# leoelm/Bayesian_inference_for_NN

Hardware: NVIDIA B200
Metric: posterior_grad_evals_per_s (higher is better)
Workload: dtype f32 (tensor-core products on two int8 fixed-point slices per operand, kind::i8, exact int32 accumulate; f32 everywhere else)

## Files before the change

### bayesian_inference_for_nn_b200/csrc/tc_fused.cuh

```cuda
#pragma once
#include "tc_layer2.cuh"

namespace pyb {

constexpr int TF_THREADS = 384;
template <int CP> struct TfCfg {
  static constexpr int STAGES = 5;
  static constexpr int W2_BYTES = 2 * 256 * CP * 4;
  static constexpr int ZX_BYTES = 2 * CP * 128 * 4;
  static constexpr int SMEM = STAGES * TP_STAGE_BYTES + 1024  + 1024  + 2048  +
                              128  + W2_BYTES + ZX_BYTES;
  static constexpr int SMEM_I8 = SMEM + 4096;
};
__device__ __forceinline__ void tc_ld_16x256b_x4_raw(uint32_t taddr, uint32_t* r) {
  asm volatile(
      "tcgen05.ld.sync.aligned.16x256b.x4.b32 "
      "{%0, %1, %2, %3, %4, %5, %6, %7, %8, %9, %10, %11, %12, %13, %14, %15}, [%16];"
      : "=r"(r[0]), "=r"(r[1]), "=r"(r[2]), "=r"(r[3]), "=r"(r[4]), "=r"(r[5]), "=r"(r[6]), "=r"(r[7]), "=r"(r[8]),
        "=r"(r[9]), "=r"(r[10]), "=r"(r[11]), "=r"(r[12]), "=r"(r[13]), "=r"(r[14]), "=r"(r[15])
      : "r"(taddr)
      : "memory");
}
__device__ __forceinline__ void tc_mma_i8_pair(uint32_t tmem_d, uint64_t adesc, uint64_t bdesc, uint32_t idesc,
                                               uint32_t accumulate) {
  asm volatile(
      "{\n"
      ".reg .pred p;\n"
      "setp.ne.b32 p, %4, 0;\n"
      "tcgen05.mma.cta_group::2.kind::i8 [%0], %1, %2, %3, p;\n"
      "}\n" ::"r"(tmem_d),
      "l"(adesc), "l"(bdesc), "r"(idesc), "r"(accumulate)
      : "memory");
}
__device__ __forceinline__ void slice4_i8(const float* d, float zq, uint32_t& hw, uint32_t& lw) {
  constexpr float M = 12582912.0f;
  uint32_t hb[4], lb[4];
#pragma unroll
  for (int r = 0; r < 4; ++r) {
    const float t = fmaf(d[r], zq, M);
    const float h = t - M;
    const float e = fmaf(d[r], zq, -h);
    const float u = fmaf(e, 254.0f, M);
    hb[r] = __float_as_uint(t);
    lb[r] = __float_as_uint(u);
  }
  hw = __byte_perm(__byte_perm(hb[0], hb[1], 0x0040), __byte_perm(hb[2], hb[3], 0x0040), 0x5410);
  lw = __byte_perm(__byte_perm(lb[0], lb[1], 0x0040), __byte_perm(lb[2], lb[3], 0x0040), 0x5410);
}

__device__ __forceinline__ void tc_ld_16x256b_x4(uint32_t taddr, float* v) {
  uint32_t r[16];
  asm volatile(
      "tcgen05.ld.sync.aligned.16x256b.x4.b32 "
      "{%0, %1, %2, %3, %4, %5, %6, %7, %8, %9, %10, %11, %12, %13, %14, %15}, [%16];"
      : "=r"(r[0]), "=r"(r[1]), "=r"(r[2]), "=r"(r[3]), "=r"(r[4]), "=r"(r[5]), "=r"(r[6]), "=r"(r[7]), "=r"(r[8]),
        "=r"(r[9]), "=r"(r[10]), "=r"(r[11]), "=r"(r[12]), "=r"(r[13]), "=r"(r[14]), "=r"(r[15])
      : "r"(taddr)
      : "memory");
#pragma unroll
  for (int i = 0; i < 16; ++i) v[i] = __uint_as_float(r[i]);
}
template <int CP>
__device__ __forceinline__ int w2_slot(int h, int c) {
  return ((((h >> 3) * 2 + (h & 1)) * (CP / 4) + (c >> 2)) * 4 + ((h >> 1) & 3)) * 4 + (c & 3);
}
__device__ __forceinline__ void split_pair(float x0, float x1, uint32_t& hw, uint32_t& lw) {
  const __nv_bfloat162 hp = __floats2bfloat162_rn(x0, x1);
  hw = *reinterpret_cast<const uint32_t*>(&hp);
  const __nv_bfloat162 lp = __floats2bfloat162_rn(x0 - __uint_as_float(hw << 16), x1 - __uint_as_float(hw & 0xffff0000u));
  lw = *reinterpret_cast<const uint32_t*>(&lp);
}

template <int CP, bool FWD, int I8 = 0>
__global__ void __cluster_dims__(2, 1, 1) __launch_bounds__(TF_THREADS, 1)
tc_g1_layer2_fused(const __grid_constant__ CUtensorMap tmA_hi, const __grid_constant__ CUtensorMap tmA_lo,
                   const __grid_constant__ CUtensorMap tmB_hi, const __grid_constant__ CUtensorMap tmB_lo,
                   const TcGemmParams p, const Layer2Params l2) {
  constexpr int STAGES = TfCfg<CP>::STAGES;
  extern __shared__ uint8_t smem_raw[];
  uint8_t* smem = smem_raw + ((1024u - (smem_u32(smem_raw) & 1023u)) & 1023u);
  uint8_t* stage_base = smem;
  uint64_t* bars = (uint64_t*)(smem + STAGES * TP_STAGE_BYTES);
  uint64_t* full_bar = bars;
  uint64_t* empty_bar = bars + STAGES;
  uint64_t* tmem_full = bars + 2 * STAGES;
  uint64_t* tmem_empty = bars + 2 * STAGES + 2;
  uint32_t* tmem_ptr = (uint32_t*)(bars + 2 * STAGES + 4);
  float* bias_s = (float*)(smem + STAGES * TP_STAGE_BYTES + 1024);
  float* b2_s = bias_s + 512;
  float* W2_s = b2_s + 32;
  float* zx_s = W2_s + 2 * 256 * CP;
  float* cw_s = zx_s + 2 * CP * 128;
  float* zq_s = cw_s + 512;

  const int warp = __shfl_sync(0xffffffffu, (int)(threadIdx.x >> 5), 0), lane = threadIdx.x & 31;
  const uint32_t rank = cluster_ctarank();
  const int cluster_id = blockIdx.x >> 1, n_clusters = gridDim.x >> 1;
  constexpr int KSTAGE = I8 ? 64 : TC_BK;
  const int nk = (p.K + KSTAGE - 1) / KSTAGE;
  const int H = p.H;
  const int half_rows = H >> 1;
  const uint32_t cta_bytes = 2 * TC_A_TILE_BYTES + 2 * (uint32_t)half_rows * TC_BK * 2;

  if (warp == 8 && lane == 0) {
    asm volatile("prefetch.tensormap [%0];" ::"l"(&tmA_hi) : "memory");
    asm volatile("prefetch.tensormap [%0];" ::"l"(&tmA_lo) : "memory");
    asm volatile("prefetch.tensormap [%0];" ::"l"(&tmB_hi) : "memory");
    asm volatile("prefetch.tensormap [%0];" ::"l"(&tmB_lo) : "memory");
  }
  if (warp == 9 && lane == 0) {
    for (int s = 0; s < STAGES; ++s) { mbar_init(&full_bar[s], 1); mbar_init(&empty_bar[s], 1); }
    mbar_init(&tmem_full[0], 1); mbar_init(&tmem_full[1], 1);
    mbar_init(&tmem_empty[0], 16); mbar_init(&tmem_empty[1], 16);
    asm volatile("fence.mbarrier_init.release.cluster;" ::: "memory");
  }
  if (warp == 10) {
    asm volatile("tcgen05.alloc.cta_group::2.sync.aligned.shared::cta.b32 [%0], %1;" ::"r"(smem_u32(tmem_ptr)), "r"(512)
                 : "memory");
    asm volatile("tcgen05.relinquish_alloc_permit.cta_group::2.sync.aligned;" ::: "memory");
  }
  tc_fence_before();
  __syncthreads();
  cluster_sync_all();
  tc_fence_after();
  const uint32_t tmem_base = *tmem_ptr;

  if (warp >= 8) {
   asm volatile("setmaxnreg.dec.sync.aligned.u32 40;");
   if (warp == 8) {
    if (lane == 0) {
      int stage = 0;
      uint32_t phase = 0;
      for (int item = cluster_id; item < p.total_items; item += n_clusters) {
        int b, mp, split;
        tc_decode(p, item, b, mp, split);
        const int arow = p.a_row0 + (mp * 2 + (int)rank) * 128;
        const int brow = b * H + (int)rank * half_rows;
        for (int kc = 0; kc < nk; ++kc) {
          (I8 ? mbar_wait_sleep(&empty_bar[stage], phase ^ 1) : mbar_wait(&empty_bar[stage], phase ^ 1));
          uint8_t* st = stage_base + stage * TP_STAGE_BYTES;
          if (rank == 0) mbar_expect_tx(&full_bar[stage], 2 * cta_bytes);
          const int k0 = kc * KSTAGE;
          tma_load_2d_pair(st, &tmA_hi, &full_bar[stage], k0, arow);
          tma_load_2d_pair(st + TC_A_TILE_BYTES, &tmA_lo, &full_bar[stage], k0, arow);
          tma_load_2d_pair(st + 2 * TC_A_TILE_BYTES, &tmB_hi, &full_bar[stage], k0, brow);
          tma_load_2d_pair(st + 2 * TC_A_TILE_BYTES + 8192, &tmB_lo, &full_bar[stage], k0, brow);
          if (++stage == STAGES) { stage = 0; phase ^= 1; }
        }
      }
    }
  } else if (warp == 9) {
    if (rank == 0 && lane == 0) {
      const uint32_t idesc = (I8 ? (2u << 4) : (1u << 4)) | (1u << 7) | (1u << 10) | ((uint32_t)(H >> 3) << 17) | ((256u >> 4) << 24);
      int stage = 0, it = 0;
      uint32_t phase = 0;
      const int k_tail = p.K - (nk - 1) * KSTAGE;
      for (int item = cluster_id; item < p.total_items; item += n_clusters, ++it) {
        const int acc = I8 ? 0 : (it & 1);
        const uint32_t acc_phase = I8 ? (uint32_t)(it & 1) : (uint32_t)((it >> 1) & 1);
        (I8 ? mbar_wait_sleep(&tmem_empty[acc], acc_phase ^ 1) : mbar_wait(&tmem_empty[acc], acc_phase ^ 1));
        tc_fence_after();
        const uint32_t d = tmem_base + (uint32_t)acc * 256;
        for (int kc = 0; kc < nk; ++kc) {
          (I8 ? mbar_wait_sleep(&full_bar[stage], phase) : mbar_wait(&full_bar[stage], phase));
          tc_fence_after();
          const uint32_t st = smem_u32(stage_base + stage * TP_STAGE_BYTES);
          const int nks = (kc == nk - 1 && k_tail <= KSTAGE / 2) ? 1 : 2;
          for (int ks = 0; ks < nks; ++ks) {
            const uint32_t koff = ks * 32;
            const uint64_t ah = make_smem_desc_sw64(st + koff);
            const uint64_t al = make_smem_desc_sw64(st + TC_A_TILE_BYTES + koff);
            const uint64_t bh = make_smem_desc_sw64(st + 2 * TC_A_TILE_BYTES + koff);
            const uint64_t bl = make_smem_desc_sw64(st + 2 * TC_A_TILE_BYTES + 8192 + koff);
            const uint32_t accum = (kc != 0) || (ks != 0);
            if (I8) {
              tc_mma_i8_pair(d, ah, bh, idesc, accum);
              tc_mma_i8_pair(d + 256, ah, bl, idesc, accum);
              tc_mma_i8_pair(d + 256, al, bh, idesc, 1);
            } else {
              tc_mma_bf16_pair(d, ah, bh, idesc, accum);
              tc_mma_bf16_pair(d, al, bh, idesc, 1);
              tc_mma_bf16_pair(d, ah, bl, idesc, 1);
            }
          }
          tc_commit_pair(&empty_bar[stage]);
          if (++stage == STAGES) { stage = 0; phase ^= 1; }
        }
        tc_commit_pair(&tmem_full[acc]);
      }
    }
   }
  } else {
    asm volatile("setmaxnreg.inc.sync.aligned.u32 232;");
    const int half = warp >> 2;
    const int quad = warp & 3;
    const int g = lane >> 2, t = lane & 3;
    const int eall = threadIdx.x;
    const uint32_t lane_addr = (uint32_t)(quad * 32) << 16;
    const int Hh = H >> 1;
    const int C = l2.C;
    const float invN = l2.scale / (float)l2.N;
    const int r_own = 2 * (t & 1) + (t >> 1);
    const int row_own = quad * 32 + g + 8 * r_own;
    const int pos0 = quad * 32 + 4 * g;
    const int hbase = half * Hh + 2 * t;
    uint16_t* z2_hi = reinterpret_cast<uint16_t*>(l2.z2_hi);
    uint16_t* z2_lo = reinterpret_cast<uint16_t*>(l2.z2_lo);
    for (int i = eall; i < 2 * 256 * CP; i += 256) W2_s[i] = 0.f;
    if (eall < 32) b2_s[eall] = 0.f;
    asm volatile("bar.sync 1, 256;" ::: "memory");
    auto fetch_consts = [&](int item, int buf) {
      int b, mp, split;
      tc_decode(p, item, b, mp, split);
      const float* th = l2.theta + (int64_t)b * l2.P;
      if (eall < H) {
        const int h = eall;
        const float* src = th + l2.w2_off + (int64_t)h * C;
        const uint32_t dst = smem_u32(W2_s + buf * 256 * CP + w2_slot<CP>(h, 0));
#pragma unroll
        for (int c = 0; c < CP; ++c)
          if (c < C)
            asm volatile("cp.async.ca.shared.global [%0], [%1], 4;" ::"r"(dst + (uint32_t)(((c >> 2) * 16 + (c & 3)) * 4)),
                         "l"(src + c) : "memory");
        asm volatile("cp.async.ca.shared.global [%0], [%1], 4;" ::"r"(smem_u32(bias_s + buf * 256 + h)),
                     "l"(p.bias + (int64_t)b * p.bias_stride + h) : "memory");
      }
      if (eall < C)
        asm volatile("cp.async.ca.shared.global [%0], [%1], 4;" ::"r"(smem_u32(b2_s + buf * 16 + eall)),
                     "l"(th + l2.b2_off + eall) : "memory");
      if (I8 && eall < H) {
        asm volatile("cp.async.ca.shared.global [%0], [%1], 4;" ::"r"(smem_u32(cw_s + buf * 256 + eall)),
                     "l"(l2.cw + (int64_t)b * H + eall) : "memory");
        if (I8 == 2 && !FWD)
          asm volatile("cp.async.ca.shared.global [%0], [%1], 4;" ::"r"(smem_u32(zq_s + buf * 256 + eall)),
                       "l"(l2.zq + (int64_t)b * H + eall) : "memory");
      }
    };
    if (cluster_id < p.total_items) fetch_consts(cluster_id, 0);
    int it = 0;
    for (int item = cluster_id; item < p.total_items; item += n_clusters, ++it) {
      int b, mp, split;
      tc_decode(p, item, b, mp, split);
      const int mt = mp * 2 + (int)rank;
      const int cbuf = it & 1;
      const int acc = I8 ? 0 : cbuf;
      const uint32_t acc_phase = I8 ? (uint32_t)(it & 1) : (uint32_t)((it >> 1) & 1);
      float* bs = bias_s + cbuf * 256;
      float* b2b = b2_s + cbuf * 16;
      float* W2b = W2_s + cbuf * 256 * CP;
      float sxr[4] = {0.f, 0.f, 0.f, 0.f};
      if (I8) {
#pragma unroll
        for (int r = 0; r < 4; ++r) {
          const int rg = mt * 128 + quad * 32 + g + 8 * r;
          sxr[r] = rg < p.M_valid ? __ldg(l2.sx + rg) : 0.f;
        }
      }
      asm volatile("cp.async.wait_all;" ::: "memory");
      asm volatile("bar.sync 1, 256;" ::: "memory");
      (I8 ? mbar_wait_sleep(&tmem_full[acc], acc_phase) : mbar_wait(&tmem_full[acc], acc_phase));
      tc_fence_after();
      const int64_t blk_w = (((((int64_t)b * p.out_tiles + mt) * H) + hbase) * 128 + pos0) >> 2;
      uint2* pa_hi = reinterpret_cast<uint2*>(p.out_hi) + blk_w;
      uint2* pa_lo = reinterpret_cast<uint2*>(p.out_lo) + blk_w;
      uint2* pz_hi = reinterpret_cast<uint2*>(l2.zt_hi) + blk_w;
      uint2* pz_lo = reinterpret_cast<uint2*>(l2.zt_lo) + blk_w;
      const float4* w4b = reinterpret_cast<const float4*>(W2b) + (((half * Hh) >> 3) * 2 * (CP / 4)) * 4 + t;
      const float* bsb = bs + hbase;
      const float* cwb = cw_s + cbuf * 256 + hbase;
      const float* zqb = zq_s + cbuf * 256 + hbase;
      uint32_t* pzi_hi = nullptr; uint32_t* pzi_lo = nullptr;
      if (I8 == 2 && !FWD) {
        const int64_t blk_b = ((((int64_t)b * p.out_tiles + mt) * H) + hbase) * 128 + pos0;
        pzi_hi = reinterpret_cast<uint32_t*>(l2.zi_hi + blk_b);
        pzi_lo = reinterpret_cast<uint32_t*>(l2.zi_lo + blk_b);
      }
      float2 z[4][CP / 2];
#pragma unroll
      for (int r = 0; r < 4; ++r)
#pragma unroll
        for (int c = 0; c < CP / 2; ++c) z[r][c] = make_float2(0.f, 0.f);
      uint32_t mask[4] = {0u, 0u, 0u, 0u};
#pragma unroll
      for (int ch = 0; ch < 4; ++ch) {
        if (ch * 32 < Hh) {
          const uint32_t col = (uint32_t)(acc * 256 + half * Hh + ch * 32);
          float v[32];
          if (I8) {
#pragma unroll
            for (int hf = 0; hf < 2; ++hf) {
              uint32_t rh[16], rc[16];
              tc_ld_16x256b_x4_raw(tmem_base + lane_addr + ((uint32_t)(16 * hf) << 16) + col, rh);
              tc_ld_16x256b_x4_raw(tmem_base + lane_addr + ((uint32_t)(16 * hf) << 16) + 256u + col, rc);
              asm volatile("tcgen05.wait::ld.sync.aligned;" ::: "memory");
#pragma unroll
              for (int j = 0; j < 16; ++j)
                v[16 * hf + j] = fmaf((float)(int)rc[j], 1.0f / 254.0f, (float)(int)rh[j]);
            }
          } else {
            tc_ld_16x256b_x4(tmem_base + lane_addr + col, v);
            tc_ld_16x256b_x4(tmem_base + lane_addr + (16u << 16) + col, v + 16);
            asm volatile("tcgen05.wait::ld.sync.aligned;" ::: "memory");
          }
          uint32_t m = 0u;
#pragma unroll
          for (int kb = 0; kb < 4; ++kb) {
            const float2 bb = *reinterpret_cast<const float2*>(bsb + ch * 32 + 8 * kb);
            float2 cc = make_float2(0.f, 0.f);
            if (I8) cc = *reinterpret_cast<const float2*>(cwb + ch * 32 + 8 * kb);
            float a[4][2];
#pragma unroll
            for (int r = 0; r < 4; ++r) {
              const float* vv = v + (r >> 1) * 16 + kb * 4 + (r & 1) * 2;
              if (I8) {
                a[r][0] = fmaxf(fmaf(vv[0], sxr[r] * cc.x, bb.x), 0.f);
                a[r][1] = fmaxf(fmaf(vv[1], sxr[r] * cc.y, bb.y), 0.f);
              } else {
                a[r][0] = fmaxf(vv[0] + bb.x, 0.f);
                a[r][1] = fmaxf(vv[1] + bb.y, 0.f);
              }
              if (!FWD) {
                m |= (a[r][0] > 0.f ? 1u : 0u) << (kb * 8 + r * 2);
                m |= (a[r][1] > 0.f ? 1u : 0u) << (kb * 8 + r * 2 + 1);
              }
            }
#pragma unroll
            for (int i = 0; i < 2; ++i) {
              const float4* w4 = w4b + (((ch * 4 + kb) * 2 + i) * (CP / 4)) * 4;
#pragma unroll
              for (int c4 = 0; c4 < CP / 4; ++c4) {
                const float4 w = w4[c4 * 4];
                const float2 w01 = make_float2(w.x, w.y), w23 = make_float2(w.z, w.w);
#pragma unroll
                for (int r = 0; r < 4; ++r) {
                  const float2 aa = make_float2(a[r][i], a[r][i]);
                  z[r][2 * c4] = __ffma2_rn(aa, w01, z[r][2 * c4]);
                  z[r][2 * c4 + 1] = __ffma2_rn(aa, w23, z[r][2 * c4 + 1]);
                }
              }
              if (!FWD) {
                uint32_t hw0, lw0, hw1, lw1;
                split_pair(a[0][i], a[1][i], hw0, lw0);
                split_pair(a[2][i], a[3][i], hw1, lw1);
                const int w_off = (ch * 32 + 8 * kb + i) * 32;
                __stcs(pa_hi + w_off, make_uint2(hw0, hw1));
                __stcs(pa_lo + w_off, make_uint2(lw0, lw1));
              }
            }
          }
          mask[ch] = m;
        }
      }
      tc_fence_before();
      __syncwarp();
      if (lane == 0) mbar_arrive_leader_relaxed(&tmem_empty[acc]);
      if (item + n_clusters < p.total_items) fetch_consts(item + n_clusters, cbuf ^ 1);
      float zo[CP];
      {
        const bool b0 = t & 1, b1 = t & 2;
#pragma unroll
        for (int c = 0; c < CP; ++c) {
          const float z0 = (c & 1) ? z[0][c >> 1].y : z[0][c >> 1].x, z1 = (c & 1) ? z[1][c >> 1].y : z[1][c >> 1].x;
          const float z2v = (c & 1) ? z[2][c >> 1].y : z[2][c >> 1].x, z3 = (c & 1) ? z[3][c >> 1].y : z[3][c >> 1].x;
          float k0 = b0 ? z2v : z0, k1 = b0 ? z3 : z1;
          const float g0 = __shfl_xor_sync(0xffffffffu, b0 ? z0 : z2v, 1);
          const float g1 = __shfl_xor_sync(0xffffffffu, b0 ? z1 : z3, 1);
          k0 = b0 ? g0 + k0 : k0 + g0;
          k1 = b0 ? g1 + k1 : k1 + g1;
          const float kk = b1 ? k1 : k0;
          const float gg = __shfl_xor_sync(0xffffffffu, b1 ? k0 : k1, 2);
          zo[c] = b1 ? gg + kk : kk + gg;
        }
      }
#pragma unroll
      for (int c = 0; c < CP; ++c) zx_s[(half * CP + c) * 128 + row_own] = zo[c];
      asm volatile("bar.sync 2, 256;" ::: "memory");
      float zf[CP], dz[CP];
#pragma unroll
      for (int c = 0; c < CP; ++c) zf[c] = (b2b[c] + zx_s[c * 128 + row_own]) + zx_s[(CP + c) * 128 + row_own];
      const int row_g = mt * 128 + row_own;
      if (FWD) {
        if (half == 0 && row_g < p.M_valid) {
          float* o = l2.fwd_out + ((int64_t)b * l2.N + row_g) * C;
          if (l2.out_act == PYB_ACT_SOFTMAX) {
            float mx = -INFINITY;
#pragma unroll
            for (int c = 0; c < CP; ++c) if (c < C) mx = fmaxf(mx, zf[c]);
            float se = 0.f;
#pragma unroll
            for (int c = 0; c < CP; ++c) if (c < C) se += expf(zf[c] - mx);
            const float inv = 1.0f / se;
#pragma unroll
            for (int c = 0; c < CP; ++c) if (c < C) o[c] = expf(zf[c] - mx) * inv;
          } else {
#pragma unroll
            for (int c = 0; c < CP; ++c) if (c < C) o[c] = act_apply(zf[c], l2.out_act);
          }
        }
        continue;
      }
      float loss_r = 0.f;
      l2_loss_dz<CP>(l2, row_g, row_g < p.M_valid, zf, dz, loss_r, invN);
      if (half == 0) {
        const int64_t blk2 = (((int64_t)b * p.out_tiles + mt) * L2_CMAX) * 128 + pos0 + r_own;
#pragma unroll
        for (int c = 0; c < CP; ++c) {
          __nv_bfloat16 hb, lb;
          split_bf16(dz[c], hb, lb);
          z2_hi[blk2 + c * 128] = __bfloat16_as_ushort(hb);
          z2_lo[blk2 + c * 128] = __bfloat16_as_ushort(lb);
        }
        const int64_t grp = (int64_t)b * l2.n_groups + mt * 4 + quad;
        float mine = 0.f;
#pragma unroll
        for (int c = 0; c < CP; ++c) {
          const float sm = warp_sum(dz[c]);
          if (lane == c) mine = sm;
        }
        if (lane < CP) l2.b2_partial[grp * L2_CMAX + lane] = mine;
        const float ls = warp_sum(loss_r);
        if (lane == 0) l2.loss_partial[grp] = (double)ls;
      }
      float2 dzp[4][CP / 2];
#pragma unroll
      for (int r = 0; r < 4; ++r) {
        const int src = (lane & ~3) | ((r >> 1) | ((r & 1) << 1));
#pragma unroll
        for (int c = 0; c < CP / 2; ++c) {
          dzp[r][c].x = __shfl_sync(0xffffffffu, dz[2 * c], src);
          dzp[r][c].y = __shfl_sync(0xffffffffu, dz[2 * c + 1], src);
        }
      }
#pragma unroll
      for (int ch = 0; ch < 4; ++ch) {
        if (ch * 32 < Hh) {
          const uint32_t m = mask[ch];
#pragma unroll
          for (int kb = 0; kb < 4; ++kb) {
#pragma unroll
            for (int i = 0; i < 2; ++i) {
              const float4* w4 = w4b + (((ch * 4 + kb) * 2 + i) * (CP / 4)) * 4;
              float2 s[4];
#pragma unroll
              for (int r = 0; r < 4; ++r) s[r] = make_float2(0.f, 0.f);
#pragma unroll
              for (int c4 = 0; c4 < CP / 4; ++c4) {
                const float4 w = w4[c4 * 4];
                const float2 w01 = make_float2(w.x, w.y), w23 = make_float2(w.z, w.w);
#pragma unroll
                for (int r = 0; r < 4; ++r) {
                  s[r] = __ffma2_rn(dzp[r][2 * c4], w01, s[r]);
                  s[r] = __ffma2_rn(dzp[r][2 * c4 + 1], w23, s[r]);
                }
              }
              float d[4];
#pragma unroll
              for (int r = 0; r < 4; ++r) d[r] = ((m >> (kb * 8 + r * 2 + i)) & 1u) ? s[r].x + s[r].y : 0.f;
              const int w_off = (ch * 32 + 8 * kb + i) * 32;
              if (I8 == 2) {
                uint32_t hw, lw;
                slice4_i8(d, zqb[ch * 32 + 8 * kb + i], hw, lw);
                __stcs(pzi_hi + w_off, hw);
                __stcs(pzi_lo + w_off, lw);
              } else {
                uint32_t hw0, lw0, hw1, lw1;
                split_pair(d[0], d[1], hw0, lw0);
                split_pair(d[2], d[3], hw1, lw1);
                __stcs(pz_hi + w_off, make_uint2(hw0, hw1));
                __stcs(pz_lo + w_off, make_uint2(lw0, lw1));
              }
            }
          }
        }
      }
    }
  }
  tc_fence_before();
  __syncthreads();
  cluster_sync_all();
  if (warp == 10) {
    tc_fence_after();
    asm volatile("tcgen05.dealloc.cta_group::2.sync.aligned.b32 %0, %1;" ::"r"(tmem_base), "r"(512) : "memory");
  }
}

}
```

### bayesian_inference_for_nn_b200/csrc/tc_path.cu

```cuda
#include <cstdlib>
#include <cstring>
#include "tc_fused_mma.cuh"
#include <algorithm>

namespace pyb {

typedef CUresult (*PFN_encodeTiled)(CUtensorMap*, CUtensorMapDataType, cuuint32_t, void*, const cuuint64_t*,
                                    const cuuint64_t*, const cuuint32_t*, const cuuint32_t*, CUtensorMapInterleave,
                                    CUtensorMapSwizzle, CUtensorMapL2promotion, CUtensorMapFloatOOBfill);
static PFN_encodeTiled get_encode() {
  static PFN_encodeTiled fn = nullptr;
  if (!fn) {
    void* f = nullptr;
    cudaDriverEntryPointQueryResult q;
    PYB_CUDA(cudaGetDriverEntryPoint("cuTensorMapEncodeTiled", &f, cudaEnableDefault, &q));
    PYB_REQUIRE(f != nullptr && q == cudaDriverEntryPointSuccess, PYB_ERR_CUDA, "cuTensorMapEncodeTiled unavailable");
    fn = (PFN_encodeTiled)f;
  }
  return fn;
}
static CUtensorMap make_map_blocked(const void* base, int64_t blocks, int rows_per_block, int box_rows) {
  CUtensorMap m;
  cuuint64_t dims[3] = {128, (cuuint64_t)rows_per_block, (cuuint64_t)blocks};
  cuuint64_t strides[2] = {256, (cuuint64_t)rows_per_block * 256};
// ... 134 lines not shown
  if (p.n_btiles > 0) return p.a_blocked && p.n_mtiles == 2 && (p.H % 16) == 0;
  if ((p.H % 32) != 0) return false;
  return !p.a_blocked && p.a_batch_rows == 0;
}
static void launch_gemm_tc(pyb_handle* h, const CUtensorMap& a_hi, const CUtensorMap& a_lo,
                           const CUtensorMap& b_hi, const CUtensorMap& b_lo, TcGemmParams p, double flops,
                           const CUtensorMap* bp_hi = nullptr, const CUtensorMap* bp_lo = nullptr) {
  if (p.k_splits <= 1) { p.k_splits = 1; p.chunks_per_split = (p.K + TC_BK - 1) / TC_BK; p.split_stride = 0; }
  p.vec_store = p.epi == EPI_STORE && ((uintptr_t)p.out % 16 == 0) && (p.out_stride % 4 == 0) && (p.out_ld % 4 == 0) &&
                (p.split_stride % 4 == 0);
  int grid = std::min(p.total_items, h->sm_count);
  prof_begin(h);
  if (bp_hi && bp_lo && pair_ok(h, p) && p.n_btiles > 1 && p.epi == EPI_STORE && p.transpose_out && h->opt_tc_dual &&
      p.H <= 256 && (p.H / 2) * TC_BK * 2 <= 8192) {
    p.total_items = p.n_batch * p.k_splits * ((p.n_btiles + 1) / 2);
    grid = std::min(2 * p.total_items, (h->sm_count / 2) * 2);
    PYB_CUDA(cudaFuncSetAttribute(tc_gemm_pair_dual_bf16x3, cudaFuncAttributeMaxDynamicSharedMemorySize, TD_SMEM_BYTES));
    tc_gemm_pair_dual_bf16x3<<<grid, TP_THREADS, TD_SMEM_BYTES, h->stream>>>(a_hi, a_lo, *bp_hi, *bp_lo, p);
    prof_end(h, flops);
    count_launch(h);
    return;
  }
  if (bp_hi && bp_lo && pair_ok(h, p)) {
    grid = std::min(2 * p.total_items, (h->sm_count / 2) * 2);
    if (p.epi == EPI_STORE) launch_pair_inst<EPI_STORE, 0>(h, grid, a_hi, a_lo, *bp_hi, *bp_lo, p);
    else if (p.act == PYB_ACT_RELU) launch_pair_inst<EPI_BIAS_ACT_T_SPLIT, PYB_ACT_RELU>(h, grid, a_hi, a_lo, *bp_hi, *bp_lo, p);
    else if (p.act == PYB_ACT_TANH) launch_pair_inst<EPI_BIAS_ACT_T_SPLIT, PYB_ACT_TANH>(h, grid, a_hi, a_lo, *bp_hi, *bp_lo, p);
    else if (p.act == PYB_ACT_SIGMOID) launch_pair_inst<EPI_BIAS_ACT_T_SPLIT, PYB_ACT_SIGMOID>(h, grid, a_hi, a_lo, *bp_hi, *bp_lo, p);
    else launch_pair_inst<EPI_BIAS_ACT_T_SPLIT, PYB_ACT_LINEAR>(h, grid, a_hi, a_lo, *bp_hi, *bp_lo, p);
    prof_end(h, flops);
    count_launch(h);
    return;
  }
  if (p.epi == EPI_STORE) launch_gemm_inst<EPI_STORE, 0>(h, grid, a_hi, a_lo, b_hi, b_lo, p);
  else if (p.act == PYB_ACT_RELU) launch_gemm_inst<EPI_BIAS_ACT_T_SPLIT, PYB_ACT_RELU>(h, grid, a_hi, a_lo, b_hi, b_lo, p);
  else if (p.act == PYB_ACT_TANH) launch_gemm_inst<EPI_BIAS_ACT_T_SPLIT, PYB_ACT_TANH>(h, grid, a_hi, a_lo, b_hi, b_lo, p);
  else if (p.act == PYB_ACT_SIGMOID) launch_gemm_inst<EPI_BIAS_ACT_T_SPLIT, PYB_ACT_SIGMOID>(h, grid, a_hi, a_lo, b_hi, b_lo, p);
  else launch_gemm_inst<EPI_BIAS_ACT_T_SPLIT, PYB_ACT_LINEAR>(h, grid, a_hi, a_lo, b_hi, b_lo, p);
  prof_end(h, flops);
  count_launch(h);
}


template <int CP, bool FWD, int I8>
static void launch_fused_i8(pyb_handle* h, int grid, const CUtensorMap& a_hi, const CUtensorMap& a_lo,
                            const CUtensorMap& b_hi, const CUtensorMap& b_lo, const TcGemmParams& p, const Layer2Params& l2) {
  PYB_CUDA(cudaFuncSetAttribute(tc_g1_layer2_fused<CP, FWD, I8>, cudaFuncAttributeMaxDynamicSharedMemorySize, TfCfg<CP>::SMEM_I8));
  tc_g1_layer2_fused<CP, FWD, I8><<<grid, TF_THREADS, TfCfg<CP>::SMEM_I8, h->stream>>>(a_hi, a_lo, b_hi, b_lo, p, l2);
}
template <int CP>
static void launch_fused_inst(pyb_handle* h, int grid, const CUtensorMap& a_hi, const CUtensorMap& a_lo,
                              const CUtensorMap& b_hi, const CUtensorMap& b_lo, const TcGemmParams& p, const Layer2Params& l2,
                              int i8 = 0) {
  if (i8 && !l2.fwd_out && h->opt_tc_epi_mma) {
    if (i8 >= 2) {
      PYB_CUDA(cudaFuncSetAttribute(tc_fused_i8_mma<CP, true>, cudaFuncAttributeMaxDynamicSharedMemorySize, TfmCfg::SMEM));
      tc_fused_i8_mma<CP, true><<<grid, TFM_THREADS, TfmCfg::SMEM, h->stream>>>(a_hi, a_lo, b_hi, b_lo, p, l2);
    } else {
      PYB_CUDA(cudaFuncSetAttribute(tc_fused_i8_mma<CP, false>, cudaFuncAttributeMaxDynamicSharedMemorySize, TfmCfg::SMEM));
      tc_fused_i8_mma<CP, false><<<grid, TFM_THREADS, TfmCfg::SMEM, h->stream>>>(a_hi, a_lo, b_hi, b_lo, p, l2);
    }
    return;
  }
  if (i8) {
    if (l2.fwd_out) launch_fused_i8<CP, true, 1>(h, grid, a_hi, a_lo, b_hi, b_lo, p, l2);
    else if (i8 >= 2) launch_fused_i8<CP, false, 2>(h, grid, a_hi, a_lo, b_hi, b_lo, p, l2);
    else launch_fused_i8<CP, false, 1>(h, grid, a_hi, a_lo, b_hi, b_lo, p, l2);
    return;
  }
  if (l2.fwd_out) {
    PYB_CUDA(cudaFuncSetAttribute(tc_g1_layer2_fused<CP, true>, cudaFuncAttributeMaxDynamicSharedMemorySize, TfCfg<CP>::SMEM));
    tc_g1_layer2_fused<CP, true><<<grid, TF_THREADS, TfCfg<CP>::SMEM, h->stream>>>(a_hi, a_lo, b_hi, b_lo, p, l2);
    return;
  }
  PYB_CUDA(cudaFuncSetAttribute(tc_g1_layer2_fused<CP, false>, cudaFuncAttributeMaxDynamicSharedMemorySize, TfCfg<CP>::SMEM));
  tc_g1_layer2_fused<CP, false><<<grid, TF_THREADS, TfCfg<CP>::SMEM, h->stream>>>(a_hi, a_lo, b_hi, b_lo, p, l2);
}
static bool fused_ok(const pyb_handle* h, int H, int act1) {
  return h->opt_tc_pair && h->opt_tc_fuse && act1 == PYB_ACT_RELU && (H == 128 || H == 256);
}

static int i8_mode(const pyb_handle* h, bool backward, bool resident) {
  const Model& m = h->model;
  int want = h->opt_tc_i8;
  if (want < 0) want = (resident && backward && h->i8_guard_ok) ? 2 : 0;
  if (want <= 0 || !fused_ok(h, m.layer[0].fan_out, m.layer[0].act) || m.layer[1].fan_out > L2_CMAX) return 0;
  if (m.layer[0].fan_in > 32768) return 0;
  if (!backward) return 1;
  const bool ce = h->loss_kind == PYB_LOSS_SPARSE_CE && m.layer[1].act == PYB_ACT_SOFTMAX;
  return (want >= 2 && ce && m.layer[0].fan_out == 256) ? 2 : 1;
}

static void tc_prepare_data_i8(pyb_handle* h, TcData& d, const float* X, int64_t N, int mode) {
  const int D = d.D;
  const int64_t Npad = d.Npad;
  d.Dk = (D + 15) / 16 * 16;
  d.col_mean.alloc(D); d.col_absmax.alloc(D); d.sx.alloc(N); d.sf.alloc(D + 1);
  d.xs_hi.alloc(N * d.Dk); d.xs_lo.alloc(N * d.Dk);
  d.stat_sum.alloc((size_t)I8_STAT_CHUNKS * D); d.stat_max.alloc((size_t)I8_STAT_CHUNKS * D);
  k_col_stats<<<dim3((D + 31) / 32, I8_STAT_CHUNKS), dim3(32, 32), 0, h->stream>>>(X, N, D, d.stat_sum.p, d.stat_max.p);
  k_col_stats_final<<<(D + 255) / 256, 256, 0, h->stream>>>(d.stat_sum.p, d.stat_max.p, I8_STAT_CHUNKS, N, D, d.col_mean.p,
                                                           d.col_absmax.p);
  count_launch(h);
  const int wpb = 8;
  k_slice_x_rows_i8<<<(unsigned)std::min<int64_t>((N + wpb - 1) / wpb, 8 * (int64_t)h->sm_count), wpb * 32, 0, h->stream>>>(
      X, N, D, d.col_mean.p, d.xs_hi.p, d.xs_lo.p, d.sx.p, d.Dk);
  count_launch(h, 2);
  d.mXs_hi = make_map_u8p(d.xs_hi.p, d.Dk, N, d.Dk, 128);
  d.mXs_lo = make_map_u8p(d.xs_lo.p, d.Dk, N, d.Dk, 128);
  if (mode >= 2) {
    d.xts_hi.alloc((int64_t)(D + 1) * Npad); d.xts_lo.alloc((int64_t)(D + 1) * Npad);
    PYB_CUDA(cudaMemsetAsync(d.xts_hi.p, 0, (size_t)(D + 1) * Npad, h->stream));
    PYB_CUDA(cudaMemsetAsync(d.xts_lo.p, 0, (size_t)(D + 1) * Npad, h->stream));
    dim3 g2((D + 31) / 32, (unsigned)((N + 31) / 32), 1), blk(32, 8);
    k_slice_xt_i8<<<g2, blk, 0, h->stream>>>(X, N, D, d.col_absmax.p, d.xts_hi.p, d.xts_lo.p, Npad);
// ... 89 lines not shown
    PYB_CUDA(cudaStreamSynchronize(h->stream));
    st->cap_chains_i8 = std::max(st->cap_chains_i8, bc);
    const int64_t cc = st->cap_chains_i8, Dk = (D + 15) / 16 * 16;
    st->ws_hi.alloc(cc * H * Dk); st->ws_lo.alloc(cc * H * Dk);
    st->cw.alloc(cc * H); st->b1c.alloc(cc * H); st->zq.alloc(cc * H); st->zd.alloc(cc * H);
    st->mWs_hi = make_map_u8p(st->ws_hi.p, Dk, cc * H, Dk, H / 2);
    st->mWs_lo = make_map_u8p(st->ws_lo.p, Dk, cc * H, Dk, H / 2);
    if (mode >= 2) {
      st->cap_blocks_i8 = std::max(st->cap_blocks_i8, need_blocks);
      const int64_t cb = st->cap_blocks_i8;
      st->zi_hi.alloc(cb * H * 128); st->zi_lo.alloc(cb * H * 128);
      st->mZi_hi = make_map_blocked_u8(st->zi_hi.p, cb, H, 128);
      st->mZi_lo = make_map_blocked_u8(st->zi_lo.p, cb, H, 128);
    }
  }
  return bc;
}

static void tc_pack_and_g1(pyb_handle* h, TcState* st, TcData& d, const float* th, int nb,
                           const Layer2Params* fused = nullptr, int i8 = 0) {
  const Model& m = h->model;
  const LayerDesc& L1 = m.layer[0];
  const int D = st->D, H = st->H;
  const int64_t N = d.N, Npad = d.Npad, P = m.P;
  if (i8) {
    const float invN = fused->fwd_out ? 1.0f : fused->scale / (float)fused->N;
    k_pack_w1_i8<<<dim3((H + 31) / 32, nb), dim3(32, 8), 0, h->stream>>>(
        th, P, L1.w_off, L1.b_off, m.layer[1].w_off, D, H, m.layer[1].fan_out, d.col_mean.p, invN, st->ws_hi.p, st->ws_lo.p,
        d.Dk, st->cw.p, st->b1c.p, st->zq.p, st->zd.p);
  } else {
  dim3 g((H + 31) / 32, (D + 31) / 32, nb), blk(32, 8);
  k_split_transpose<<<g, blk, 0, h->stream>>>(th + L1.w_off, P, D, H, H, st->w_hi.p, st->w_lo.p, (int64_t)H * D, D);
  }
  count_launch(h);
  TcGemmParams p = {};
  p.K = D; p.n_mtiles = (int)(Npad / 128); p.n_pairs = (p.n_mtiles + 1) / 2; p.n_batch = nb; p.H = H;
  p.a_batch_rows = 0; p.a_box_rows = 128; p.order = 1; p.sub_batch = 32; p.total_items = p.n_pairs * nb;
  p.epi = EPI_BIAS_ACT_T_SPLIT;
  p.bias = th + L1.b_off; p.bias_stride = P; p.act = L1.act;
  p.out_hi = st->a_hi.p; p.out_lo = st->a_lo.p; p.out_tiles = (int)(Npad / 128);
  p.M_valid = (int)N; p.N_valid = H;
  if (fused) {
    const int grid = std::min(2 * p.total_items, (h->sm_count / 2) * 2);
    const int C = fused->C;
    Layer2Params f2 = *fused;
    const CUtensorMap &a_hi = i8 ? d.mXs_hi : d.mX_hi, &a_lo = i8 ? d.mXs_lo : d.mX_lo;
    const CUtensorMap &b_hi = i8 ? st->mWs_hi : st->mWp_hi, &b_lo = i8 ? st->mWs_lo : st->mWp_lo;
    if (i8) {
      p.bias = st->b1c.p; p.bias_stride = H;
      f2.dbg = nullptr; f2.dbg_flags = h->opt_tc_timeline & ~1;
      if (h->opt_tc_timeline) { st->dbg.alloc(8 * 160); f2.dbg = st->dbg.p; }
      f2.sx = d.sx.p; f2.cw = st->cw.p; f2.zq = st->zq.p; f2.zi_hi = st->zi_hi.p; f2.zi_lo = st->zi_lo.p;
    }
    prof_begin(h);
    if (C <= 4) launch_fused_inst<4>(h, grid, a_hi, a_lo, b_hi, b_lo, p, f2, i8);
    else if (C <= 8) launch_fused_inst<8>(h, grid, a_hi, a_lo, b_hi, b_lo, p, f2, i8);
    else if (C <= 12) launch_fused_inst<12>(h, grid, a_hi, a_lo, b_hi, b_lo, p, f2, i8);
    else launch_fused_inst<16>(h, grid, a_hi, a_lo, b_hi, b_lo, p, f2, i8);
    prof_end(h, 2.0 * N * (D * (double)H + (fused->fwd_out ? 1.0 : 3.0) * H * C) * nb);
    count_launch(h);
    return;
  }
  launch_gemm_tc(h, d.mX_hi, d.mX_lo, st->mW_hi, st->mW_lo, p, 2.0 * N * D * (double)H * nb, &st->mWp_hi, &st->mWp_lo);
}

static void tc_eval_on(pyb_handle* h, TcState* st, TcData& d, const int32_t* y_i, const float* y_f, const float* theta,
                       int64_t S, float scale, float* loss_out, float* grad_out) {
  const Model& m = h->model;
  const int64_t Bc = tc_prepare_bufs(h, st, S, d.Npad, true, d.i8);
  const LayerDesc& L1 = m.layer[0];
  const LayerDesc& L2 = m.layer[1];
  const int D = st->D, H = st->H, C = st->C;
  const int64_t N = d.N, Npad = d.Npad, P = m.P;
  const int n_tiles = (int)(Npad / L2_ROWS);
  const bool fused = fused_ok(h, H, L1.act) && C <= L2_CMAX;
  const int i8 = d.i8;
  const int n_groups = fused ? (int)(Npad / 128) * 4
                             : std::min(n_tiles, std::max(1, (int)((8 * (int64_t)h->sm_count + Bc - 1) / Bc)));
  st->b2_partial.alloc((size_t)Bc * n_groups * L2_CMAX);
  st->loss_partial.alloc((size_t)Bc * n_groups);
  for (int64_t b0 = 0; b0 < S; b0 += Bc) {
    const int nb = (int)std::min<int64_t>(Bc, S - b0);
    const float* th = theta + b0 * P;
    float* gr = grad_out + b0 * P;
    {
      Layer2Params p = {};
      p.a_hi = st->a_hi.p; p.a_lo = st->a_lo.p; p.zt_hi = st->z_hi.p; p.zt_lo = st->z_lo.p;
      p.z2_hi = st->z2_hi.p; p.z2_lo = st->z2_lo.p; p.k_tiles = (int)(Npad / 128);
      p.theta = th; p.P = P; p.w2_off = L2.w_off; p.b2_off = L2.b_off;
      p.H = H; p.C = C; p.N = (int)N; p.act1 = L1.act; p.out_act = L2.act; p.loss_kind = h->loss_kind;
      p.y_i = y_i; p.y_f = y_f; p.scale = scale;
      p.loss_partial = st->loss_partial.p; p.b2_partial = st->b2_partial.p; p.n_groups = n_groups;
      p.n_tiles = n_tiles;
      if (fused) {
        tc_pack_and_g1(h, st, d, th, nb, &p, i8);
      } else {
        tc_pack_and_g1(h, st, d, th, nb);
        dim3 g(n_groups, nb);
        if (C <= 4) k_layer2<4><<<g, 128, 0, h->stream>>>(p);
        else if (C <= 8) k_layer2<8><<<g, 128, 0, h->stream>>>(p);
        else if (C <= 12) k_layer2<12><<<g, 128, 0, h->stream>>>(p);
        else k_layer2<16><<<g, 128, 0, h->stream>>>(p);
      }
      k_layer2_reduce<<<nb, 256, 0, h->stream>>>(st->b2_partial.p, st->loss_partial.p, n_groups, C, gr, P, L2.b_off,
                                                loss_out ? loss_out + b0 : nullptr, (int)N);
      count_launch(h, 2);
    }
    const int nk_rows = (int)(Npad / TC_BK);
    const int splits = (nk_rows + TC_SPLIT_CHUNKS - 1) / TC_SPLIT_CHUNKS;
// ... 288 lines not shown
```

Before: 10940.

## Pipeline per-block TMEM loads in fused epilogue and add a ten-class instance

The fused layer-2 epilogue now reads TMEM in small 8-column blocks and issues the next block's load while computing on the current one. The TMEM-empty arrive moves to right after the last block is read, so the MMA warp can start the next item earlier. A CP=10 template instance with padded W2 shared-memory strides (CPS) and a tail pair path is added, so ten-class models do no wasted work on padding classes out to 12. Optional clock-based timeline instrumentation is added behind the debug pointer. The cost is more frequent load/wait round trips and a more complex register schedule.

```diff
diff --git a/bayesian_inference_for_nn_b200/csrc/tc_fused.cuh b/bayesian_inference_for_nn_b200/csrc/tc_fused.cuh
--- a/bayesian_inference_for_nn_b200/csrc/tc_fused.cuh
+++ b/bayesian_inference_for_nn_b200/csrc/tc_fused.cuh
@@ -6,7 +6,8 @@
 constexpr int TF_THREADS = 384;
 template <int CP> struct TfCfg {
   static constexpr int STAGES = 5;
-  static constexpr int W2_BYTES = 2 * 256 * CP * 4;
+  static constexpr int CPS = (CP + 3) / 4 * 4;
+  static constexpr int W2_BYTES = 2 * 256 * CPS * 4;
   static constexpr int ZX_BYTES = 2 * CP * 128 * 4;
   static constexpr int SMEM = STAGES * TP_STAGE_BYTES + 1024  + 1024  + 2048  +
                               128  + W2_BYTES + ZX_BYTES;
@@ -48,17 +49,11 @@
   lw = __byte_perm(__byte_perm(lb[0], lb[1], 0x0040), __byte_perm(lb[2], lb[3], 0x0040), 0x5410);
 }
 
-__device__ __forceinline__ void tc_ld_16x256b_x4(uint32_t taddr, float* v) {
-  uint32_t r[16];
-  asm volatile(
-      "tcgen05.ld.sync.aligned.16x256b.x4.b32 "
-      "{%0, %1, %2, %3, %4, %5, %6, %7, %8, %9, %10, %11, %12, %13, %14, %15}, [%16];"
-      : "=r"(r[0]), "=r"(r[1]), "=r"(r[2]), "=r"(r[3]), "=r"(r[4]), "=r"(r[5]), "=r"(r[6]), "=r"(r[7]), "=r"(r[8]),
-        "=r"(r[9]), "=r"(r[10]), "=r"(r[11]), "=r"(r[12]), "=r"(r[13]), "=r"(r[14]), "=r"(r[15])
-      : "r"(taddr)
-      : "memory");
-#pragma unroll
-  for (int i = 0; i < 16; ++i) v[i] = __uint_as_float(r[i]);
+__device__ __forceinline__ void tc_ld_16x256b_x1_raw(uint32_t taddr, uint32_t* r) {
+  asm volatile("tcgen05.ld.sync.aligned.16x256b.x1.b32 {%0, %1, %2, %3}, [%4];"
+               : "=r"(r[0]), "=r"(r[1]), "=r"(r[2]), "=r"(r[3])
+               : "r"(taddr)
+               : "memory");
 }
 template <int CP>
 __device__ __forceinline__ int w2_slot(int h, int c) {
@@ -77,6 +72,8 @@
                    const __grid_constant__ CUtensorMap tmB_hi, const __grid_constant__ CUtensorMap tmB_lo,
                    const TcGemmParams p, const Layer2Params l2) {
   constexpr int STAGES = TfCfg<CP>::STAGES;
+  constexpr int CPS = TfCfg<CP>::CPS;
+  static_assert(CP % 2 == 0, "classes are processed in pairs");
   extern __shared__ uint8_t smem_raw[];
   uint8_t* smem = smem_raw + ((1024u - (smem_u32(smem_raw) & 1023u)) & 1023u);
   uint8_t* stage_base = smem;
@@ -89,7 +86,7 @@
   float* bias_s = (float*)(smem + STAGES * TP_STAGE_BYTES + 1024);
   float* b2_s = bias_s + 512;
   float* W2_s = b2_s + 32;
-  float* zx_s = W2_s + 2 * 256 * CP;
+  float* zx_s = W2_s + 2 * 256 * CPS;
   float* cw_s = zx_s + 2 * CP * 128;
   float* zq_s = cw_s + 512;
 
@@ -155,15 +152,22 @@
       int stage = 0, it = 0;
       uint32_t phase = 0;
       const int k_tail = p.K - (nk - 1) * KSTAGE;
+      const bool tl = l2.dbg != nullptr;
+      uint32_t t_wait = 0, t_loop = 0, t_fill = 0, c1 = 0;
       for (int item = cluster_id; item < p.total_items; item += n_clusters, ++it) {
         const int acc = I8 ? 0 : (it & 1);
         const uint32_t acc_phase = I8 ? (uint32_t)(it & 1) : (uint32_t)((it >> 1) & 1);
+        if (tl) c1 = (uint32_t)clock();
         (I8 ? mbar_wait_sleep(&tmem_empty[acc], acc_phase ^ 1) : mbar_wait(&tmem_empty[acc], acc_phase ^ 1));
         tc_fence_after();
+        if (tl) { const uint32_t c = (uint32_t)clock(); t_wait += c - c1; c1 = c; }
         const uint32_t d = tmem_base + (uint32_t)acc * 256;
         for (int kc = 0; kc < nk; ++kc) {
+          uint32_t f0 = 0;
+          if (tl) f0 = (uint32_t)clock();
           (I8 ? mbar_wait_sleep(&full_bar[stage], phase) : mbar_wait(&full_bar[stage], phase));
           tc_fence_after();
+          if (tl) t_fill += (uint32_t)clock() - f0;
           const uint32_t st = smem_u32(stage_base + stage * TP_STAGE_BYTES);
           const int nks = (kc == nk - 1 && k_tail <= KSTAGE / 2) ? 1 : 2;
           for (int ks = 0; ks < nks; ++ks) {
@@ -187,6 +191,13 @@
           if (++stage == STAGES) { stage = 0; phase ^= 1; }
         }
         tc_commit_pair(&tmem_full[acc]);
+        if (tl) t_loop += (uint32_t)clock() - c1;
+      }
+      if (tl) {
+        l2.dbg[blockIdx.x * 8 + 0] = (unsigned long long)t_wait;
+        l2.dbg[blockIdx.x * 8 + 1] = (unsigned long long)t_loop;
+        l2.dbg[blockIdx.x * 8 + 2] = (unsigned long long)t_fill;
+        l2.dbg[blockIdx.x * 8 + 3] = (unsigned long long)it;
       }
     }
    }
@@ -206,7 +217,7 @@
     const int hbase = half * Hh + 2 * t;
     uint16_t* z2_hi = reinterpret_cast<uint16_t*>(l2.z2_hi);
     uint16_t* z2_lo = reinterpret_cast<uint16_t*>(l2.z2_lo);
-    for (int i = eall; i < 2 * 256 * CP; i += 256) W2_s[i] = 0.f;
+    for (int i = eall; i < 2 * 256 * CPS; i += 256) W2_s[i] = 0.f;
     if (eall < 32) b2_s[eall] = 0.f;
     asm volatile("bar.sync 1, 256;" ::: "memory");
     auto fetch_consts = [&](int item, int buf) {
@@ -216,7 +227,7 @@
       if (eall < H) {
         const int h = eall;
         const float* src = th + l2.w2_off + (int64_t)h * C;
-        const uint32_t dst = smem_u32(W2_s + buf * 256 * CP + w2_slot<CP>(h, 0));
+        const uint32_t dst = smem_u32(W2_s + buf * 256 * CPS + w2_slot<CPS>(h, 0));
 #pragma unroll
         for (int c = 0; c < CP; ++c)
           if (c < C)
@@ -237,8 +248,14 @@
       }
     };
     if (cluster_id < p.total_items) fetch_consts(cluster_id, 0);
+    const bool tl = l2.dbg != nullptr;
+    uint32_t e_top = 0, e_wait = 0, e_A = 0, e_x = 0, e_sm = 0, e_B = 0, tp = 0;
+    auto lap = [&](uint32_t& sum) {
+      if (tl) { const uint32_t c = (uint32_t)clock(); sum += c - tp; tp = c; }
+    };
     int it = 0;
     for (int item = cluster_id; item < p.total_items; item += n_clusters, ++it) {
+      if (tl) tp = (uint32_t)clock();
       int b, mp, split;
       tc_decode(p, item, b, mp, split);
       const int mt = mp * 2 + (int)rank;
@@ -247,7 +264,7 @@
       const uint32_t acc_phase = I8 ? (uint32_t)(it & 1) : (uint32_t)((it >> 1) & 1);
       float* bs = bias_s + cbuf * 256;
       float* b2b = b2_s + cbuf * 16;
-      float* W2b = W2_s + cbuf * 256 * CP;
+      float* W2b = W2_s + cbuf * 256 * CPS;
       float sxr[4] = {0.f, 0.f, 0.f, 0.f};
       if (I8) {
 #pragma unroll
@@ -258,14 +275,16 @@
       }
       asm volatile("cp.async.wait_all;" ::: "memory");
       asm volatile("bar.sync 1, 256;" ::: "memory");
+      lap(e_top);
       (I8 ? mbar_wait_sleep(&tmem_full[acc], acc_phase) : mbar_wait(&tmem_full[acc], acc_phase));
       tc_fence_after();
+      lap(e_wait);
       const int64_t blk_w = (((((int64_t)b * p.out_tiles + mt) * H) + hbase) * 128 + pos0) >> 2;
       uint2* pa_hi = reinterpret_cast<uint2*>(p.out_hi) + blk_w;
       uint2* pa_lo = reinterpret_cast<uint2*>(p.out_lo) + blk_w;
       uint2* pz_hi = reinterpret_cast<uint2*>(l2.zt_hi) + blk_w;
       uint2* pz_lo = reinterpret_cast<uint2*>(l2.zt_lo) + blk_w;
-      const float4* w4b = reinterpret_cast<const float4*>(W2b) + (((half * Hh) >> 3) * 2 * (CP / 4)) * 4 + t;
+      const float4* w4b = reinterpret_cast<const float4*>(W2b) + (((half * Hh) >> 3) * 2 * (CPS / 4)) * 4 + t;
       const float* bsb = bs + hbase;
       const float* cwb = cw_s + cbuf * 256 + hbase;
       const float* zqb = zq_s + cbuf * 256 + hbase;
@@ -275,43 +294,53 @@
         pzi_hi = reinterpret_cast<uint32_t*>(l2.zi_hi + blk_b);
         pzi_lo = reinterpret_cast<uint32_t*>(l2.zi_lo + blk_b);
       }
+      const int nblk = Hh >> 3;
+      uint32_t rw[4][4];
+      auto load_blk = [&](int s) {
+        const uint32_t ta = tmem_base + lane_addr + (uint32_t)(acc * 256 + half * Hh + 8 * s);
+        tc_ld_16x256b_x1_raw(ta, rw[0]);
+        tc_ld_16x256b_x1_raw(ta + (16u << 16), rw[2]);
+        if (I8) {
+          tc_ld_16x256b_x1_raw(ta + 256u, rw[1]);
+          tc_ld_16x256b_x1_raw(ta + (16u << 16) + 256u, rw[3]);
+        }
+      };
       float2 z[4][CP / 2];
 #pragma unroll
       for (int r = 0; r < 4; ++r)
 #pragma unroll
         for (int c = 0; c < CP / 2; ++c) z[r][c] = make_float2(0.f, 0.f);
       uint32_t mask[4] = {0u, 0u, 0u, 0u};
+      load_blk(0);
+      asm volatile("tcgen05.wait::ld.sync.aligned;" ::: "memory");
 #pragma unroll
       for (int ch = 0; ch < 4; ++ch) {
         if (ch * 32 < Hh) {
-          const uint32_t col = (uint32_t)(acc * 256 + half * Hh + ch * 32);
-          float v[32];
-          if (I8) {
-#pragma unroll
-            for (int hf = 0; hf < 2; ++hf) {
-              uint32_t rh[16], rc[16];
-              tc_ld_16x256b_x4_raw(tmem_base + lane_addr + ((uint32_t)(16 * hf) << 16) + col, rh);
-              tc_ld_16x256b_x4_raw(tmem_base + lane_addr + ((uint32_t)(16 * hf) << 16) + 256u + col, rc);
-              asm volatile("tcgen05.wait::ld.sync.aligned;" ::: "memory");
-#pragma unroll
-              for (int j = 0; j < 16; ++j)
-                v[16 * hf + j] = fmaf((float)(int)rc[j], 1.0f / 254.0f, (float)(int)rh[j]);
+          uint32_t m = 0u;
+#pragma unroll
+          for (int kb = 0; kb < 4; ++kb) {
+            const int blk = ch * 4 + kb;
+            float v[8];
+#pragma unroll
+            for (int hf = 0; hf < 2; ++hf)
+#pragma unroll
+              for (int j = 0; j < 4; ++j)
+                v[4 * hf + j] = I8 ? fmaf((float)(int)rw[2 * hf + 1][j], 1.0f / 254.0f, (float)(int)rw[2 * hf][j])
+                                   : __uint_as_float(rw[2 * hf][j]);
+            if (blk + 1 < nblk) {
+              load_blk(blk + 1);
+            } else {
+              tc_fence_before();
+              __syncwarp();
+              if (lane == 0) mbar_arrive_leader_relaxed(&tmem_empty[acc]);
             }
-          } else {
-            tc_ld_16x256b_x4(tmem_base + lane_addr + col, v);
-            tc_ld_16x256b_x4(tmem_base + lane_addr + (16u << 16) + col, v + 16);
-            asm volatile("tcgen05.wait::ld.sync.aligned;" ::: "memory");
-          }
-          uint32_t m = 0u;
-#pragma unroll
-          for (int kb = 0; kb < 4; ++kb) {
             const float2 bb = *reinterpret_cast<const float2*>(bsb + ch * 32 + 8 * kb);
             float2 cc = make_float2(0.f, 0.f);
             if (I8) cc = *reinterpret_cast<const float2*>(cwb + ch * 32 + 8 * kb);
             float a[4][2];
 #pragma unroll
             for (int r = 0; r < 4; ++r) {
-              const float* vv = v + (r >> 1) * 16 + kb * 4 + (r & 1) * 2;
+              const float* vv = v + (r >> 1) * 4 + (r & 1) * 2;
               if (I8) {
                 a[r][0] = fmaxf(fmaf(vv[0], sxr[r] * cc.x, bb.x), 0.f);
                 a[r][1] = fmaxf(fmaf(vv[1], sxr[r] * cc.y, bb.y), 0.f);
@@ -326,7 +355,7 @@
             }
 #pragma unroll
             for (int i = 0; i < 2; ++i) {
-              const float4* w4 = w4b + (((ch * 4 + kb) * 2 + i) * (CP / 4)) * 4;
+              const float4* w4 = w4b + (((ch * 4 + kb) * 2 + i) * (CPS / 4)) * 4;
 #pragma unroll
               for (int c4 = 0; c4 < CP / 4; ++c4) {
                 const float4 w = w4[c4 * 4];
@@ -337,6 +366,11 @@
                   z[r][2 * c4] = __ffma2_rn(aa, w01, z[r][2 * c4]);
                   z[r][2 * c4 + 1] = __ffma2_rn(aa, w23, z[r][2 * c4 + 1]);
                 }
+              }
+              if (CP % 4) {
+                const float2 wt = *reinterpret_cast<const float2*>(w4 + (CP / 4) * 4);
+#pragma unroll
+                for (int r = 0; r < 4; ++r) z[r][CP / 2 - 1] = __ffma2_rn(make_float2(a[r][i], a[r][i]), wt, z[r][CP / 2 - 1]);
               }
               if (!FWD) {
                 uint32_t hw0, lw0, hw1, lw1;
@@ -347,13 +381,12 @@
                 __stcs(pa_lo + w_off, make_uint2(lw0, lw1));
               }
             }
+            if (blk + 1 < nblk) asm volatile("tcgen05.wait::ld.sync.aligned;" ::: "memory");
           }
           mask[ch] = m;
         }
       }
-      tc_fence_before();
-      __syncwarp();
-      if (lane == 0) mbar_arrive_leader_relaxed(&tmem_empty[acc]);
+      lap(e_A);
       if (item + n_clusters < p.total_items) fetch_consts(item + n_clusters, cbuf ^ 1);
       float zo[CP];
       {
@@ -375,6 +408,7 @@
 #pragma unroll
       for (int c = 0; c < CP; ++c) zx_s[(half * CP + c) * 128 + row_own] = zo[c];
       asm volatile("bar.sync 2, 256;" ::: "memory");
+      lap(e_x);
       float zf[CP], dz[CP];
 #pragma unroll
       for (int c = 0; c < CP; ++c) zf[c] = (b2b[c] + zx_s[c * 128 + row_own]) + zx_s[(CP + c) * 128 + row_own];
@@ -431,6 +465,7 @@
           dzp[r][c].y = __shfl_sync(0xffffffffu, dz[2 * c + 1], src);
         }
       }
+      lap(e_sm);
 #pragma unroll
       for (int ch = 0; ch < 4; ++ch) {
         if (ch * 32 < Hh) {
@@ -439,7 +474,7 @@
           for (int kb = 0; kb < 4; ++kb) {
 #pragma unroll
             for (int i = 0; i < 2; ++i) {
-              const float4* w4 = w4b + (((ch * 4 + kb) * 2 + i) * (CP / 4)) * 4;
+              const float4* w4 = w4b + (((ch * 4 + kb) * 2 + i) * (CPS / 4)) * 4;
               float2 s[4];
 #pragma unroll
               for (int r = 0; r < 4; ++r) s[r] = make_float2(0.f, 0.f);
@@ -452,6 +487,11 @@
                   s[r] = __ffma2_rn(dzp[r][2 * c4], w01, s[r]);
                   s[r] = __ffma2_rn(dzp[r][2 * c4 + 1], w23, s[r]);
                 }
+              }
+              if (CP % 4) {
+                const float2 wt = *reinterpret_cast<const float2*>(w4 + (CP / 4) * 4);
+#pragma unroll
+                for (int r = 0; r < 4; ++r) s[r] = __ffma2_rn(dzp[r][CP / 2 - 1], wt, s[r]);
               }
               float d[4];
 #pragma unroll
@@ -473,6 +513,17 @@
           }
         }
       }
+      lap(e_B);
+    }
+    if (tl && warp == 0 && lane == 0) {
+      if (blockIdx.x & 1) {
+        l2.dbg[blockIdx.x * 8 + 0] = (unsigned long long)e_x;
+        l2.dbg[blockIdx.x * 8 + 1] = (unsigned long long)e_sm;
+      }
+      l2.dbg[blockIdx.x * 8 + 4] = (unsigned long long)e_top;
+      l2.dbg[blockIdx.x * 8 + 5] = (unsigned long long)e_wait;
+      l2.dbg[blockIdx.x * 8 + 6] = (unsigned long long)e_A;
+      l2.dbg[blockIdx.x * 8 + 7] = (unsigned long long)e_B;
     }
   }
   tc_fence_before();
diff --git a/bayesian_inference_for_nn_b200/csrc/tc_path.cu b/bayesian_inference_for_nn_b200/csrc/tc_path.cu
--- a/bayesian_inference_for_nn_b200/csrc/tc_path.cu
+++ b/bayesian_inference_for_nn_b200/csrc/tc_path.cu
@@ -210,15 +210,17 @@
 static void launch_fused_inst(pyb_handle* h, int grid, const CUtensorMap& a_hi, const CUtensorMap& a_lo,
                               const CUtensorMap& b_hi, const CUtensorMap& b_lo, const TcGemmParams& p, const Layer2Params& l2,
                               int i8 = 0) {
-  if (i8 && !l2.fwd_out && h->opt_tc_epi_mma) {
-    if (i8 >= 2) {
-      PYB_CUDA(cudaFuncSetAttribute(tc_fused_i8_mma<CP, true>, cudaFuncAttributeMaxDynamicSharedMemorySize, TfmCfg::SMEM));
-      tc_fused_i8_mma<CP, true><<<grid, TFM_THREADS, TfmCfg::SMEM, h->stream>>>(a_hi, a_lo, b_hi, b_lo, p, l2);
-    } else {
-      PYB_CUDA(cudaFuncSetAttribute(tc_fused_i8_mma<CP, false>, cudaFuncAttributeMaxDynamicSharedMemorySize, TfmCfg::SMEM));
-      tc_fused_i8_mma<CP, false><<<grid, TFM_THREADS, TfmCfg::SMEM, h->stream>>>(a_hi, a_lo, b_hi, b_lo, p, l2);
-    }
-    return;
+  if constexpr (CP % 4 == 0) {
+    if (i8 && !l2.fwd_out && h->opt_tc_epi_mma) {
+      if (i8 >= 2) {
+        PYB_CUDA(cudaFuncSetAttribute(tc_fused_i8_mma<CP, true>, cudaFuncAttributeMaxDynamicSharedMemorySize, TfmCfg::SMEM));
+        tc_fused_i8_mma<CP, true><<<grid, TFM_THREADS, TfmCfg::SMEM, h->stream>>>(a_hi, a_lo, b_hi, b_lo, p, l2);
+      } else {
+        PYB_CUDA(cudaFuncSetAttribute(tc_fused_i8_mma<CP, false>, cudaFuncAttributeMaxDynamicSharedMemorySize, TfmCfg::SMEM));
+        tc_fused_i8_mma<CP, false><<<grid, TFM_THREADS, TfmCfg::SMEM, h->stream>>>(a_hi, a_lo, b_hi, b_lo, p, l2);
+      }
+      return;
+    }
   }
   if (i8) {
     if (l2.fwd_out) launch_fused_i8<CP, true, 1>(h, grid, a_hi, a_lo, b_hi, b_lo, p, l2);
@@ -414,9 +416,11 @@
       if (h->opt_tc_timeline) { st->dbg.alloc(8 * 160); f2.dbg = st->dbg.p; }
       f2.sx = d.sx.p; f2.cw = st->cw.p; f2.zq = st->zq.p; f2.zi_hi = st->zi_hi.p; f2.zi_lo = st->zi_lo.p;
     }
+    const bool epi_mma = i8 && !f2.fwd_out && h->opt_tc_epi_mma;
     prof_begin(h);
     if (C <= 4) launch_fused_inst<4>(h, grid, a_hi, a_lo, b_hi, b_lo, p, f2, i8);
     else if (C <= 8) launch_fused_inst<8>(h, grid, a_hi, a_lo, b_hi, b_lo, p, f2, i8);
+    else if (C <= 10 && !epi_mma) launch_fused_inst<10>(h, grid, a_hi, a_lo, b_hi, b_lo, p, f2, i8);
     else if (C <= 12) launch_fused_inst<12>(h, grid, a_hi, a_lo, b_hi, b_lo, p, f2, i8);
     else launch_fused_inst<16>(h, grid, a_hi, a_lo, b_hi, b_lo, p, f2, i8);
     prof_end(h, 2.0 * N * (D * (double)H + (fused->fwd_out ? 1.0 : 3.0) * H * C) * nb);
```

New measurement: 11120 (median of 6 runs). 1.02x the previous value.
